# Lumina-Group/libzkp

Measured on AMD Instinct MI355X. Metric: proofs/sec (whole node) + ms/proof p50, 4096-proof mixed batch (range / equality / membership / improvement) per MI355X, higher is better.
Workload: dtype u32/u64 integer limbs (10x25.5-bit GF(2^255-19), BN254 Fq on 9x29-bit limbs in the MSM loops and 10x26-bit elsewhere, 8x32-bit Fr and scalars mod l, 2x64-bit f128)

## Files before the change

### libzkp_amd/csrc/g16_impl.inc

```

namespace {

struct G16Key {
    bool loaded = false;
    uint32_t n_inst = 0, n_wit = 0, nv = 0, n_rows = 0, m = 0, logm = 0;
    G16Circuit C{};
    std::vector<void*> allocs;
    uint32_t *table_g1 = nullptr, *table_g2 = nullptr;
    G16Radix rx = g16_radix(G16_WBITS_DEFAULT);
    int shared_tables = -1;
    uint64_t table_bytes = 0;
    struct Chunking { DevLayout lay; const uint32_t* corr = nullptr; const uint16_t* scal = nullptr; };
    std::vector<SlotList> targets_g1, targets_g2;
    std::vector<uint16_t> hscal_g1, hscal_g2;
    std::map<uint64_t, Chunking> lays_g1, lays_g2;
    uint64_t win_g1 = 0, win_g2 = 0;
    const uint32_t *init_g1 = nullptr, *init_g2 = nullptr;
    G16Vk vk{}; bool vk_ready = false;
    uint64_t vk_table_bytes = 0;
    bool verifier_only() const { return vk_ready && !loaded; }
    const uint32_t *vm_kconst = nullptr, *vm_lines = nullptr;
};
struct G16Run {
    void* buf = nullptr; size_t cap = 0; hipStream_t side = nullptr, side2 = nullptr; hipEvent_t ev[4] = {nullptr, nullptr, nullptr, nullptr};
    hipEvent_t last = nullptr; bool used = false;
};
struct G16State {
    G16Key key[2];
    uint32_t* mimc_dev = nullptr;
    G16Run run[2][2];
    bool attr_set = false;
    G16VmTables vm;
};
G16State& g16s() {
    if (!dev().g16) dev().g16 = new G16State();
    return *dev().g16;
}

template <class Tv> int dev_upload(G16Key& K, Tv** dst, const std::vector<typename std::remove_const<Tv>::type>& src) {
    typename std::remove_const<Tv>::type* p = nullptr;
    HIP_TRY(hipMalloc(&p, src.size() * sizeof(src[0]) + 16));
    if (!src.empty()) HIP_TRY(hipMemcpy(p, src.data(), src.size() * sizeof(src[0]), hipMemcpyHostToDevice));
// ... 42 lines not shown
template <class J> void append_words(std::vector<uint32_t>& v, const J& p) { const uint32_t* w = reinterpret_cast<const uint32_t*>(&p); for (size_t i = 0; i < sizeof(J) / 4; i++) v.push_back(w[i]); }
template <class J> J host_neg_multiple(const J& o, uint32_t k) {
    J acc = o; for (uint32_t i = 1; i < k; i++) acc = jac_add(acc, o);
    return jac_neg(acc);
}
void append_offset(std::vector<uint32_t>& v, bool g2, uint32_t k) {
    const MsmOffsets& o = msm_offsets();
    if (!g2) append_words(v, k ? host_neg_multiple(o.o1, k) : o.o1); else append_words(v, k ? host_neg_multiple(o.o2, k) : o.o2);
}
int upload_offset_point(G16Key& K, bool g2, const uint32_t** d_init) { std::vector<uint32_t> init; append_offset(init, g2, 0); return dev_upload(K, d_init, init); }
uint32_t choose_chunks(uint64_t windows, uint32_t ntargets, uint32_t rows, uint32_t resident, uint32_t tb) {
    const uint32_t groups = (rows + tb - 1) / tb;
    uint32_t hi = (uint32_t)(windows / 8); if (hi > 2048) hi = 2048; if (hi < ntargets) hi = ntargets;
    uint32_t best = ntargets; double best_cost = 1e300;
    for (uint32_t c = ntargets; c <= hi; c++) {
        const double rounds = std::ceil((double)c * groups / resident);
        const double cost = rounds * (std::ceil((double)windows / c) + 2.5) + 0.25 * c / 8.0;
        if (cost < best_cost) { best_cost = cost; best = c; }
    }
    return best;
}
int get_chunking(G16Key& K, bool g2, int part, uint32_t rows, const G16Key::Chunking** out) {
    const uint32_t resident = (uint32_t)dev().num_cu * g16_msm_blocks_per_cu(g2);
    if (part == G16_PART_ALL && !g2) return fail(ZKP_HIP_E_ARGUMENT, "G16_PART_ALL is the G2 launch");
    const std::vector<SlotList> targets = g16_part_targets(g2 ? K.targets_g2 : K.targets_g1, part);
    uint32_t c = choose_chunks(g16_windows(targets), (uint32_t)targets.size(), rows, resident, g16_msm_rows_per_block(g2));
    if (g_budget_request >= 10000) c = g_budget_request - 10000;
    auto& cache = g2 ? K.lays_g2 : K.lays_g1;
    const uint64_t key = (uint64_t)part << 32 | c;
    auto it = cache.find(key);
    if (it == cache.end()) {
        const G16Chunks P = g16_plan_chunks(targets, g2 ? K.hscal_g2 : K.hscal_g1, part, c);
        G16Key::Chunking ch; int rc;
        const GatherShape shape{K.rx.nent, K.rx.slot_ent, K.rx.uneven ? 1u : 0u, K.rx.digw};
        if ((rc = upload_layout(ch.lay, P.L, &shape, P.scal.data()))) return rc;
        std::vector<uint32_t> corr;
        for (uint32_t k : P.offsets) append_offset(corr, g2, k);
        if ((rc = dev_upload(K, &ch.corr, corr))) return rc;
        if ((rc = dev_upload(K, &ch.scal, P.scal))) return rc;
        it = cache.emplace(key, ch).first;
    }
    *out = &it->second;
    return 0;
}


uint64_t key_table_bytes(size_t n1, size_t n2, uint32_t wbits, bool uneven = false) {
    const G16Radix rx = g16_radix(wbits, uneven);
    return ((uint64_t)n1 * g16_table_entry_words(false, true) + (uint64_t)n2 * g16_table_entry_words(true, true)) * 4ull * rx.slot_ent;
}
int choose_radix(size_t n1, size_t n2, uint32_t* wbits_out, bool* uneven_out) {
    *uneven_out = false;
    const int forced = env_int("ZKP_HIP_G16_WBITS", 0);
    if (forced) {
        if (forced < (int)G16_WBITS_MIN || forced > (int)G16_WBITS_MAX) return fail(ZKP_HIP_E_ARGUMENT, "ZKP_HIP_G16_WBITS must be 8..15");
        *wbits_out = (uint32_t)forced; *uneven_out = forced == 14 && env_int("ZKP_HIP_G16_UNEVEN", 1) != 0; return 0;
    }
    size_t free_b = 0, total_b = 0;
    HIP_TRY(hipMemGetInfo(&free_b, &total_b));
    const int budget_mb = env_int("ZKP_HIP_G16_TABLE_BUDGET_MB", 0);
    const uint64_t reserve = 8ull << 30;
    const uint64_t fits = free_b > reserve ? (uint64_t)((free_b - reserve) * 0.45) : 0;
    uint64_t budget = budget_mb > 0 ? (uint64_t)budget_mb << 20 : fits;
    uint32_t first = G16_WBITS_KNEE;
    if (budget_mb > 0) {
        first = G16_WBITS_DEFAULT;
        if (G16_WBITS_DEFAULT == 14 && env_int("ZKP_HIP_G16_UNEVEN", 1) != 0 && key_table_bytes(n1, n2, 14, true) <= budget) { *wbits_out = 14; *uneven_out = true; return 0; }
    }
    for (uint32_t w = first; w >= G16_WBITS_MIN; w--)
        if (key_table_bytes(n1, n2, w) <= budget) { *wbits_out = w; return 0; }
    char msg[256];
    snprintf(msg, sizeof msg, "not enough device memory for the proving key's window tables: %llu MB at the smallest radix (2^%u), budget %llu MB (%llu MB free)",
             (unsigned long long)(key_table_bytes(n1, n2, G16_WBITS_MIN) >> 20), G16_WBITS_MIN, (unsigned long long)(budget >> 20), (unsigned long long)(free_b >> 20));
    return fail(ZKP_HIP_E_RUNTIME, msg);
}
struct SharedTables { int hip_dev, kind; uint8_t digest[32]; uint32_t wbits; bool share_ab; uint32_t *g1, *g2; int refs; };
struct TableRegistry { std::mutex mu; std::vector<SharedTables> v; std::map<int, std::mutex> build_mu; };
TableRegistry& table_registry() { static TableRegistry* r = new TableRegistry(); return *r; }
std::mutex& table_build_mutex(int hip_dev) { TableRegistry& R = table_registry(); std::lock_guard<std::mutex> lk(R.mu); return R.build_mu[hip_dev]; }
bool acquire_tables(G16Key& K, const SharedTables& want, bool any_radix) {
    TableRegistry& R = table_registry();
    std::lock_guard<std::mutex> lk(R.mu);
    for (size_t i = 0; i < R.v.size(); i++) {
        SharedTables& e = R.v[i];
        if (e.refs <= 0 || e.hip_dev != want.hip_dev || e.kind != want.kind || e.share_ab != want.share_ab || memcmp(e.digest, want.digest, 32) || (!any_radix && e.wbits != want.wbits)) continue;
        e.refs++; K.shared_tables = (int)i; K.table_g1 = e.g1; K.table_g2 = e.g2; K.rx = g16_radix(e.wbits & 0xffu, (e.wbits >> 8) != 0);
        return true;
    }
    return false;
}
void register_tables(G16Key& K, SharedTables e) {
    TableRegistry& R = table_registry();
    std::lock_guard<std::mutex> lk(R.mu);
    e.refs = 1; R.v.push_back(e);
    K.shared_tables = (int)R.v.size() - 1; K.table_g1 = e.g1; K.table_g2 = e.g2;
}
template <uint32_t AW, class Pt>
int build_tables(G16Key& K, const std::vector<Pt>& bases, uint32_t** table, bool msm_form, const G16Radix& rx, bool owned = true) {
    std::vector<uint32_t> flat; flat.reserve(bases.size() * AW);
    for (auto& b : bases) { const uint32_t* w = reinterpret_cast<const uint32_t*>(&b); for (uint32_t k = 0; k < AW; k++) flat.push_back(w[k]); }
    uint32_t* d_bases = nullptr; int rc;
    if ((rc = dev_upload(K, &d_bases, flat))) return rc;
    const size_t words = bases.size() * (size_t)rx.slot_ent * g16_table_entry_words(AW == 40, msm_form);
    uint32_t* tab = nullptr;
    if (hipMalloc(&tab, words * 4 + 64) != hipSuccess) {
        (void)hipGetLastError();
        char msg[200]; snprintf(msg, sizeof msg, "out of device memory allocating %llu MB of key tables (radix 2^%u)", (unsigned long long)((words * 4) >> 20), rx.wbits);
        return fail(ZKP_HIP_E_RUNTIME, msg);
    }
    if (owned) K.allocs.push_back(tab);
    g16_launch_build_table(AW == 40, d_bases, (uint32_t)bases.size(), tab, dev().stream, msm_form, rx);
    HIP_TRY(hipGetLastError());
    HIP_TRY(hipStreamSynchronize(dev().stream));
    *table = tab;
    return 0;
}

void release_key(G16Key& K) {
    (void)hipDeviceSynchronize();
    if (K.shared_tables >= 0) {
        TableRegistry& R = table_registry();
        std::lock_guard<std::mutex> lk(R.mu);
        SharedTables& e = R.v[(size_t)K.shared_tables];
        if (--e.refs == 0) { (void)hipFree(e.g1); (void)hipFree(e.g2); e.g1 = e.g2 = nullptr; }
    }
    for (void* p : K.allocs) (void)hipFree(p);
    for (auto& e : K.lays_g1) free_layout(e.second.lay);
    for (auto& e : K.lays_g2) free_layout(e.second.lay);
    K = G16Key();
}
int load_key_body(int kind, const uint8_t* pk, uint64_t len);
int no_proving_key(const G16Key& K) {
    return fail(ZKP_HIP_E_ARGUMENT, K.verifier_only() ? "only a verifying key is loaded for this circuit: proving needs the proving key (zkp_hip_groth16_load_key)"
                                                      : "no proving key loaded for this circuit (zkp_hip_groth16_load_key)");
}
int load_key_locked(int kind, const uint8_t* pk, uint64_t len) {
    if (kind != G16_EQUALITY && kind != G16_MEMBERSHIP) return fail(ZKP_HIP_E_ARGUMENT, "unknown circuit kind");
    G16Key& K = g16s().key[kind];
    if (K.loaded || K.shared_tables >= 0 || !K.allocs.empty()) release_key(K);
    int rc;
// ... 18 lines not shown
    K.vk.ml_alpha_beta = miller_loop(B.beta_g2.p, aff_neg(B.alpha_g1.p));
    std::vector<uint32_t> kc(6 * 20), lines;
    g16_vm_key_constants(B.beta_g2.p, aff_neg(B.alpha_g1.p), B.gamma_g2.p, B.delta_g2.p, kc.data(), lines);
    if ((rc = dev_upload(K, &K.vm_kconst, kc)) || (rc = dev_upload(K, &K.vm_lines, lines))) return rc;
    K.vk_ready = true;
    return 0;
}
int ensure_mimc_dev() {
    if (g16s().mimc_dev) return 0;
    ensure_mimc_constants();
    std::vector<uint32_t> mc; for (auto& c : g_mimc_host) put_fr(mc, c);
    HIP_TRY(hipMalloc(&g16s().mimc_dev, mc.size() * 4)); HIP_TRY(hipMemcpy(g16s().mimc_dev, mc.data(), mc.size() * 4, hipMemcpyHostToDevice));
    return 0;
}
int load_key_body(int kind, const uint8_t* pk, uint64_t len) {
    G16Key& K = g16s().key[kind];
    const HostR1CS cs = kind == G16_EQUALITY ? build_equality_r1cs() : build_membership_r1cs();
    int rc;
    KeyReader R{pk, len};
    G16VkBlob B; G16PkBlob Q;
    const int format = g16_read_key_prefix(R, B);
    if (format == G16_BLOB_MALFORMED)
        return fail(ZKP_HIP_E_ARGUMENT, "malformed proving key or verifying key (expected ark-serialize uncompressed ProvingKey<Bn254>, or its VerifyingKey<Bn254> alone)");
    if (format == G16_BLOB_VERIFYING_KEY) {
        if (const char* why = g16_check_verifying_key(B, cs.n_inst)) return fail(ZKP_HIP_E_ARGUMENT, why);
        return install_verifying_key(K, B);
    }
    if (const char* why = g16_read_proving_key(R, B, g16_key_shape(cs), Q)) return fail(ZKP_HIP_E_ARGUMENT, why);
    const bool share_ab = env_int("ZKP_HIP_G16_SHARE_AB", 1) != 0;
    G16KeyPlan P;
    if (const char* why = g16_plan_key(P, B, Q, cs, share_ab)) return fail(ZKP_HIP_E_UNSUPPORTED, why);
    SharedTables want{}; want.hip_dev = dev().hip_dev; want.kind = kind; want.share_ab = share_ab; sha256_host(want.digest, pk, len);
    std::lock_guard<std::mutex> build_lock(table_build_mutex(want.hip_dev));
    if (env_int("ZKP_HIP_G16_WBITS", 0) != 0 || !acquire_tables(K, want, true)) {
        uint32_t wb = 0; bool uneven = false;
        if ((rc = choose_radix(P.radix_points_g1, P.radix_points_g2, &wb, &uneven))) return rc;
        K.rx = g16_radix(wb, uneven); want.wbits = K.rx.wbits | K.rx.uneven << 8;
        if (!acquire_tables(K, want, false)) {
            if ((rc = build_tables<20>(K, P.bases_g1, &want.g1, true, K.rx, false))) return rc;
            if ((rc = build_tables<40>(K, P.bases_g2, &want.g2, true, K.rx, false))) { (void)hipFree(want.g1); return rc; }
            register_tables(K, want);
        }
    }
    K.table_bytes = key_table_bytes(P.bases_g1.size(), P.bases_g2.size(), K.rx.wbits, K.rx.uneven);
    if ((rc = upload_circuit(K, cs)) || (rc = ensure_mimc_dev())) return rc;
    K.targets_g1 = g16_plan_targets(P.cls_g1, K.rx); K.targets_g2 = g16_plan_targets(P.cls_g2, K.rx);
    K.win_g1 = g16_windows(K.targets_g1); K.win_g2 = g16_windows(K.targets_g2);
    K.hscal_g1 = P.row_g1; K.hscal_g2 = P.row_g2;
    if ((rc = upload_offset_point(K, false, &K.init_g1)) || (rc = upload_offset_point(K, true, &K.init_g2))) return rc;
    if (!g16_check_verifying_key(B, K.n_inst) && (rc = install_verifying_key(K, B))) return rc;
    K.loaded = true;
    return 0;
}


fr tape_fr(const uint32_t seed[8], uint32_t idx, uint32_t slot) { uint32_t w[16]; tape_draw64(w, seed, idx, slot); return fp_from_wide<FrParams>(w); }

MsmView g16_msm_view(const G16Radix& rx, const DevLayout& D, const uint16_t* slot_scalar, const uint32_t* table, const uint32_t* acc_init, uint32_t rows, const uint32_t* digits, uint32_t* partial) {
    MsmView m; m.nwin = rx.nwin; m.nent = rx.nent; m.digw = rx.digw; m.slot_ent = rx.slot_ent; m.uneven = rx.uneven; m.rows = rows; m.nslots = D.nslots; m.nchunks = D.nchunks; m.table = table; m.digits = digits;
    m.slot_base = D.slot_base; m.slot_scalar = slot_scalar; m.slot_nwin = D.slot_nwin; m.chunk_begin = D.chunk_begin; m.chunk_win0 = D.chunk_win0; m.chunk_nwin = D.chunk_nwin; m.partial = partial; m.acc_init = acc_init;
    m.steps = D.steps; m.chunk_step0 = D.chunk_step0;
    return m;
}

int gpu_scalar_mults(bool g2, const std::vector<fr>& scalars, std::vector<uint8_t>& out_bytes) {
    const uint32_t rows = (uint32_t)scalars.size(), AW = g2 ? 40 : 20, JW = g2 ? G2_JAC_W : G1_JAC_W, PB = g2 ? 128 : 64;
    std::vector<uint32_t> base;
    if (!g2) append_words(base, host_g1_generator()); else append_words(base, host_g2_generator());
    std::vector<uint32_t> offs; append_offset(offs, g2, 0); append_offset(offs, g2, 1);
    const G16Radix rx = g16_radix(10);
    std::vector<uint32_t> dig((size_t)rx.digw * rows);
    for (uint32_t i = 0; i < rows; i++) {
        sc raw; fp_to_raw(raw.v, scalars[i]); uint32_t pk[G16_DIGW_MAX]; g16_recode(pk, raw, rx);
        for (uint32_t k = 0; k < rx.digw; k++) dig[(size_t)k * rows + i] = pk[k];
    }
    uint32_t *d_base = nullptr, *d_tab = nullptr, *d_dig = nullptr, *d_part = nullptr, *d_offs = nullptr, *d_sums = nullptr; uint8_t* d_out = nullptr;
    DevScope mem;
    HIP_TRY(mem.alloc(&d_base, AW * 4)); HIP_TRY(mem.alloc(&d_tab, (size_t)rx.slot_ent * g16_table_entry_words(g2, true) * 4 + 64)); HIP_TRY(mem.alloc(&d_dig, dig.size() * 4));
    HIP_TRY(mem.alloc(&d_part, (size_t)JW * 4 * rows)); HIP_TRY(mem.alloc(&d_sums, (size_t)JW * 4 * rows)); HIP_TRY(mem.alloc(&d_offs, offs.size() * 4));
    HIP_TRY(hipMemcpy(d_offs, offs.data(), offs.size() * 4, hipMemcpyHostToDevice)); HIP_TRY(mem.alloc(&d_out, (size_t)PB * rows));
    HIP_TRY(hipMemcpy(d_base, base.data(), AW * 4, hipMemcpyHostToDevice));
// ... 64 lines not shown
    put_len(pk, nv); put(pk, g1at(o_a), 64ull * nv);
    put_len(pk, nv); put(pk, g1at(o_b), 64ull * nv);
    put_len(pk, nv); put(pk, g2at(3), 128ull * nv);
    put_len(pk, m - 1); put(pk, g1at(o_h), 64ull * (m - 1));
    put_len(pk, T.n_wit); put(pk, g1at(o_l), 64ull * T.n_wit);
    return load_key_locked(kind, pk.data(), pk.size());
}

int launch_msm_key(bool g2, const G16Radix& rx, const G16Key::Chunking& ch, const uint32_t* table, const uint32_t* acc_init, uint32_t rows, const uint32_t* digits, uint32_t* partial, hipStream_t st) {
    const DevLayout& D = ch.lay;
    const MsmView m = g16_msm_view(rx, D, ch.scal, table, acc_init, rows, digits, partial);
    Device::KProf& K = dev().prof[g2 ? 2 : 1];
    hipEvent_t e1 = nullptr;
    int rc = prof_begin(K, st, &e1);
    if (rc) return rc;
    ZKP_TRACED(g2 ? "k_msm_gather<G2Msm>" : "k_msm_gather<G1Msm>", st, g16_launch_msm(g2, m, st));
    prof_end(K, st, e1, D.adds_per_row * rows);
    return 0;
}


int run_g16(int kind, uint32_t rows, const uint64_t* d_value, const uint64_t* d_set_vals, const uint32_t* d_set_len, const uint8_t* d_seeds,
            uint8_t* d_out, uint64_t stride, hipStream_t st, uint32_t lane = 0) {
    G16Key& K = g16s().key[kind];
    if (!K.loaded) return no_proving_key(K);
    const uint32_t nsc = g16_nscalars(K.nv, K.m);
    const G16Key::Chunking *c1 = nullptr, *c1c = nullptr, *c2 = nullptr;
    int rc;
    if ((rc = get_chunking(K, false, G16_PART_AB, rows, &c1)) || (rc = get_chunking(K, true, G16_PART_ALL, rows, &c2))) return rc;
    if ((rc = get_chunking(K, false, G16_PART_C, rows, &c1c))) return rc;
    size_t off = 0;
    auto sz = [&](size_t bytes) { size_t o = off; off += align_up(bytes); return o; };
    const size_t W = (size_t)32 * rows;
    const size_t o_z = sz(W * K.nv), o_sd = sz((size_t)K.rx.digw * 4 * rows * nsc), o_rs = sz(W * 2), o_p1 = sz((size_t)c1->lay.nchunks * G1_JAC_W * 4 * rows),
                 o_p1c = sz((size_t)c1c->lay.nchunks * G1_JAC_W * 4 * rows), o_p2 = sz((size_t)c2->lay.nchunks * G2_JAC_W * 4 * rows),
                 o_s1 = sz((size_t)3 * G1_JAC_W * 4 * rows), o_s2 = sz((size_t)G2_JAC_W * 4 * rows), o_t1 = sz((size_t)G16_CPARTS * G1_JAC_W * 4 * rows),
                 o_qe = sz((size_t)2 * 9 * K.m * 4 * rows);
    G16Run& RW = g16s().run[kind][lane & 1u];
    if (off > RW.cap) {
        if (RW.buf) { HIP_TRY(hipDeviceSynchronize()); HIP_TRY(hipFree(RW.buf)); RW.buf = nullptr; RW.cap = 0; }
        HIP_TRY(hipMalloc(&RW.buf, off)); RW.cap = off;
    }
    uint8_t* base = (uint8_t*)RW.buf;
    G16View V{}; V.rx = K.rx; V.rows = rows; V.kind = (uint32_t)kind; V.n_inst = K.n_inst; V.n_wit = K.n_wit; V.nv = K.nv; V.m = K.m;
    V.value = d_value; V.set_vals = d_set_vals; V.set_len = d_set_len; V.seeds = reinterpret_cast<const uint32_t*>(d_seeds); V.mimc_c = g16s().mimc_dev;
    V.z = (uint32_t*)(base + o_z); V.sdig = (uint32_t*)(base + o_sd); V.rs = (uint32_t*)(base + o_rs); V.out = d_out; V.stride = stride;
    V.qap_evals = (uint32_t*)(base + o_qe);
    uint32_t *p1 = (uint32_t*)(base + o_p1), *p1c = (uint32_t*)(base + o_p1c), *p2 = (uint32_t*)(base + o_p2), *s1 = (uint32_t*)(base + o_s1), *s2 = (uint32_t*)(base + o_s2), *t1 = (uint32_t*)(base + o_t1);
    if (!RW.last) {
        for (auto& e : RW.ev) HIP_TRY(hipEventCreateWithFlags(&e, hipEventDisableTiming));
        HIP_TRY(hipEventCreateWithFlags(&RW.last, hipEventDisableTiming));
    }
    G16Run& R0 = g16s().run[kind][0];
    if (!R0.side) {
        static const int side_level = env_int("ZKP_HIP_G16_SIDE_PRIORITY", 2), side2_level = env_int("ZKP_HIP_G16_SIDE2_PRIORITY", 0);
        HIP_TRY(hipStreamCreateWithPriority(&R0.side, hipStreamNonBlocking, stream_priority(side_level)));
        HIP_TRY(hipStreamCreateWithPriority(&R0.side2, hipStreamNonBlocking, stream_priority(side2_level)));
    }
    hipStream_t const side = R0.side, side2 = R0.side2;
    hipEvent_t ev_wit = RW.ev[0], ev_ab = RW.ev[1], ev_c = RW.ev[2], ev_cp = RW.ev[3];
    ReduceView R2{}; R2.rows = rows; R2.ntargets = 1; R2.partial = p2; R2.target_chunk_begin = c2->lay.target_chunk_begin; R2.corr = c2->corr;
    if (RW.used) HIP_TRY(hipStreamWaitEvent(st, RW.last, 0));
    ZKP_TRACED("k_g16_witness", st, g16_launch_witness(V, st));
    ZKP_TRACED("k_g16_zdigits", st, g16_launch_zdigits(V, st));
    HIP_TRY(hipEventRecord(ev_wit, st));
    HIP_TRY(hipStreamWaitEvent(side, ev_wit, 0));
    { TraceMark tm_("k_g16_qap", side); HIP_TRY(g16_launch_qap(V, K.C, side)); }
    if ((rc = launch_msm_key(false, K.rx, *c1c, K.table_g1, K.init_g1, rows, V.sdig, p1c, side))) return rc;
    ReduceView Rc{}; Rc.rows = rows; Rc.ntargets = 1; Rc.partial = p1c; Rc.target_chunk_begin = c1c->lay.target_chunk_begin; Rc.corr = c1c->corr;
    ZKP_TRACED("k_sum_t<G1Msm>", side, g16_launch_sum(false, Rc, s1 + (size_t)2 * G1_JAC_W * rows, side));
    HIP_TRY(hipEventRecord(ev_c, side));
    if ((rc = launch_msm_key(false, K.rx, *c1, K.table_g1, K.init_g1, rows, V.sdig, p1, st))) return rc;
    ReduceView Rab{}; Rab.rows = rows; Rab.ntargets = 2; Rab.partial = p1; Rab.target_chunk_begin = c1->lay.target_chunk_begin; Rab.corr = c1->corr;
    if (c1->lay.ntargets == 3) Rab.target_chunk_end = c1->lay.target_chunk_begin + 2;
    HIP_TRY(hipEventRecord(ev_ab, st));
    HIP_TRY(hipStreamWaitEvent(side2, ev_ab, 0));
    ZKP_TRACED("k_sum_t<G1Msm>", side2, g16_launch_sum(false, Rab, s1, side2));
    ZKP_TRACED("k_g16_cparts", side2, g16_launch_cparts(V, s1, t1, side2));
    HIP_TRY(hipEventRecord(ev_cp, side2));
    if ((rc = launch_msm_key(true, K.rx, *c2, K.table_g2, K.init_g2, rows, V.sdig, p2, st))) return rc;
    ZKP_TRACED("k_sum_t<G2Msm>", st, g16_launch_sum(true, R2, s2, st));
    HIP_TRY(hipStreamWaitEvent(st, ev_c, 0));
    HIP_TRY(hipStreamWaitEvent(st, ev_cp, 0));
    ZKP_TRACED("k_g16_final", st, g16_launch_final(V, s1, s2, t1, st));
    HIP_TRY(hipGetLastError());
    HIP_TRY(hipEventRecord(RW.last, st)); RW.used = true;
    return 0;
}

int prove_g16_host(int kind, uint64_t n, const uint64_t* values, const uint64_t* sets_flat, const uint32_t* set_counts, const std::vector<uint8_t>& valid,
                   const uint8_t* seeds, uint8_t* out, uint64_t stride, uint32_t* out_len, int32_t* status) {
    if (g16s().key[kind].verifier_only()) return no_proving_key(g16s().key[kind]);
    std::vector<uint64_t> v, sv; std::vector<uint32_t> sl, idx; std::vector<uint8_t> sd;
    size_t pos = 0; int any = 0;
    memset(out, 0, stride * n);
    for (uint64_t i = 0; i < n; i++) {
        const uint32_t cnt = set_counts ? set_counts[i] : 0;
        if (valid[i]) {
            idx.push_back((uint32_t)i); v.push_back(values[i]);
            sd.insert(sd.end(), seeds + 32 * i, seeds + 32 * i + 32);
            if (kind == G16_MEMBERSHIP) { sl.push_back(cnt); for (uint32_t k = 0; k < G16_MAX_SET; k++) sv.push_back(k < cnt ? sets_flat[pos + k] : 0); }
            const uint32_t plen = kind == G16_EQUALITY ? 298u : 10u + 4u + 8u * cnt + 256u + 32u;
            if (plen > stride) return fail(ZKP_HIP_E_ARGUMENT, "stride too small for the proof envelope");
            out_len[i] = plen; status[i] = ZKP_HIP_OK;
        } else { out_len[i] = 0; status[i] = ZKP_HIP_INVALID_INPUT; any = 1; }
        pos += cnt;
    }
    const uint32_t rows = (uint32_t)idx.size();
    if (rows == 0) return any;
    hipStream_t st = dev().stream;
    uint64_t *d_v = nullptr, *d_sv = nullptr; uint32_t* d_sl = nullptr; uint8_t *d_sd = nullptr, *d_out = nullptr;
    DevScope mem;
    HIP_TRY(mem.alloc(&d_v, 8ull * rows)); HIP_TRY(mem.alloc(&d_sd, 32ull * rows)); HIP_TRY(mem.alloc(&d_out, stride * rows));
// ... 291 lines not shown
```

### libzkp_amd/csrc/g16_share.h

```cpp
#pragma once
#include <cstdint>
#include <vector>
#include "bp_layout.h"
#include "g16_circuit.h"
#include "g16_keyblob.h"

namespace zkp {

inline bool g16_shared_point(const G1Pt& a, const G1Pt& b) { return !a.inf && !b.inf && fq_eq(a.p.x, b.p.x) && fq_eq(a.p.y, b.p.y); }

struct G16AbSlots { SlotList a, s, b; };
inline G16AbSlots g16_ab_slots(const std::vector<G1Pt>& aq, const std::vector<G1Pt>& b1q, const std::vector<uint8_t>& cls, bool share) {
    G16AbSlots out;
    const size_t n = aq.size() < b1q.size() ? aq.size() : b1q.size();
    for (size_t k = 0; k < aq.size(); k++) {
        if (aq[k].inf) continue;
        if (share && k < n && g16_shared_point(aq[k], b1q[k])) out.s.push_back({(uint16_t)k, cls[k]});
        else out.a.push_back({(uint16_t)k, cls[k]});
    }
    for (size_t k = 0; k < b1q.size(); k++) {
        if (b1q[k].inf || (share && k < n && g16_shared_point(aq[k], b1q[k]))) continue;
        out.b.push_back({(uint16_t)k, cls[k]});
    }
    return out;
// ... 22 lines not shown
    const G16KeyShape sh = g16_key_shape(cs);
    if (sh.nv + sh.m + 3 > 65535 || 3ull * sh.nv + sh.m + 8 > 65535) return "circuit too large for 16-bit slot indices";
    const uint32_t SC_H = sh.nv, SC_R = sh.nv + sh.m - 1, SC_S = SC_R + 1, SC_NRS = SC_R + 2, SC_ONE = SC_R + 3;
    std::vector<uint8_t> cls(cs.inst_nwin); cls.insert(cls.end(), cs.wit_nwin.begin(), cs.wit_nwin.end());
    P = G16KeyPlan(); P.cls_g1.resize(4); P.cls_g2.resize(1);
    auto add1 = [&](int list, const G1Pt& pt, uint32_t row, uint8_t c) {
        if (pt.inf) return;
        P.cls_g1[list].push_back({(uint16_t)P.bases_g1.size(), c}); P.bases_g1.push_back(pt.p); P.row_g1.push_back((uint16_t)row);
    };
    auto add2 = [&](const G2Pt& pt, uint32_t row, uint8_t c) {
        if (pt.inf) return;
        P.cls_g2[0].push_back({(uint16_t)P.bases_g2.size(), c}); P.bases_g2.push_back(pt.p); P.row_g2.push_back((uint16_t)row);
    };
    const G16AbSlots ab = g16_ab_slots(pk.a_query, pk.b_g1_query, cls, share_ab);
    for (auto& sl : ab.a) add1(0, pk.a_query[sl.first], sl.first, sl.second);
    add1(0, pk.delta_g1, SC_R, G16_NW_FULL); add1(0, vk.alpha_g1, SC_ONE, 1);
    for (auto& sl : ab.s) add1(1, pk.a_query[sl.first], sl.first, sl.second);
    for (auto& sl : ab.b) add1(2, pk.b_g1_query[sl.first], sl.first, sl.second);
    add1(2, pk.delta_g1, SC_S, G16_NW_FULL); add1(2, pk.beta_g1, SC_ONE, 1);
    for (uint32_t k = 0; k < sh.n_wit; k++) add1(3, pk.l_query[k], sh.n_inst + k, cls[sh.n_inst + k]);
    for (uint32_t i = 0; i + 1 < sh.m; i++) add1(3, pk.h_query[i], SC_H + i, G16_NW_FULL);
    add1(3, pk.delta_g1, SC_NRS, G16_NW_FULL);
    for (uint32_t k = 0; k < sh.nv; k++) add2(pk.b_g2_query[k], k, cls[k]);
    add2(vk.delta_g2, SC_S, G16_NW_FULL); add2(vk.beta_g2, SC_ONE, 1);
    P.radix_points_g1 = pk.a_query.size() + pk.b_g1_query.size() - ab.s.size() + pk.l_query.size() + pk.h_query.size() + 5;
    P.radix_points_g2 = pk.b_g2_query.size() + 2;
    return nullptr;
}
inline std::vector<SlotList> g16_plan_targets(const std::vector<SlotList>& cls, const G16Radix& rx) {
    std::vector<SlotList> out = cls;
    for (auto& t : out) for (auto& sl : t) sl.second = g16_class_nwin(sl.second, rx);
    return out;
}
inline uint64_t g16_windows(const std::vector<SlotList>& targets) { uint64_t w = 0; for (auto& t : targets) for (auto& sl : t) w += sl.second; return w; }

enum { G16_PART_ALL = 0, G16_PART_AB = 1, G16_PART_C = 2 };
inline std::vector<SlotList> g16_part_targets(const std::vector<SlotList>& all, int part) {
    if (part == G16_PART_ALL) return all;
    if (part == G16_PART_AB) return g16_ab_targets(all[0], all[1], all[2]);
    return std::vector<SlotList>(all.begin() + 3, all.end());
}
struct G16Chunks { MsmLayout L; std::vector<uint16_t> scal; std::vector<uint32_t> offsets; };
inline G16Chunks g16_plan_chunks(const std::vector<SlotList>& targets, const std::vector<uint16_t>& row, int part, uint32_t chunks) {
    G16Chunks C; C.L = make_layout_even(targets, chunks);
    for (uint16_t b : C.L.slot_base) C.scal.push_back(row[b]);
    if (part == G16_PART_AB) { const G16AbRanges ab = g16_ab_ranges(C.L); for (int t = 0; t < 2; t++) C.offsets.push_back((uint32_t)ab.end[t] - ab.begin[t]); }
    else for (uint32_t t = 0; t < C.L.ntargets(); t++) C.offsets.push_back((uint32_t)C.L.target_chunk_begin[t + 1] - C.L.target_chunk_begin[t]);
    return C;
}

}
```

### libzkp_amd/csrc/g16_steps.h

```cpp
#pragma once
#include "bn254_g.h"
#include "bn254_fr9.h"
#include "keccak.h"
#include "sc25519.h"

namespace zkp {

struct G16Radix { uint32_t wbits, nwin, nent, digw, nwin_u64, uneven, slot_ent; };
constexpr uint32_t G16_UNEVEN_TOP_ENT = 25088;
ZKP_HD inline G16Radix g16_radix(uint32_t wbits, bool uneven = false) {
    G16Radix r; r.wbits = wbits; r.nwin = (254 + wbits) / wbits; r.nent = 1u << (wbits - 1); r.nwin_u64 = (64 + wbits) / wbits; r.uneven = 0;
    r.slot_ent = r.nwin * r.nent;
    if (uneven && wbits == 14) { r.uneven = 1; r.nwin = 18; r.slot_ent = 18u * r.nent + G16_UNEVEN_TOP_ENT; }
    r.digw = (r.nwin + 1) / 2;
    return r;
}
ZKP_HD inline uint32_t g16_win_bit(const G16Radix& rx, uint32_t w) { return rx.uneven && w == 17 ? 239u : rx.wbits * w; }
ZKP_HD inline uint32_t g16_win_off(const G16Radix& rx, uint32_t w) { return (w + (rx.uneven && w == 17 ? 1u : 0u)) * rx.nent; }
ZKP_HD inline uint32_t g16_win_ent(const G16Radix& rx, uint32_t w) { return !rx.uneven || w < 16 ? rx.nent : w == 16 ? 2u * rx.nent : G16_UNEVEN_TOP_ENT; }
constexpr uint32_t G16_WBITS_DEFAULT = 14, G16_WBITS_KNEE = 13, G16_WBITS_MIN = 8, G16_WBITS_MAX = 15, G16_DIGW_MAX = 16;
static_assert(G16_WBITS_DEFAULT >= G16_WBITS_MIN && G16_WBITS_DEFAULT <= G16_WBITS_MAX, "key-table radix out of range");
ZKP_HD inline void g16_recode_uneven(uint32_t* packed, const sc& raw) {
    uint32_t carry = 0;
    ZKP_UNROLL for (int j = 0; j < 18; j++) {
        const int bit = j == 17 ? 239 : 14 * j, wb = j < 16 ? 14 : 15, wd = bit >> 5, sh = bit & 31;
        uint32_t x = wd < 8 ? raw.v[wd] >> sh : 0u;
        if (sh + wb > 32 && wd + 1 < 8) x |= raw.v[wd + 1] << (32 - sh);
        uint32_t d = (x & ((1u << wb) - 1u)) + carry;
        carry = j < 17 && d > (1u << (wb - 1)) ? 1u : 0u;
        d = (d - (carry << wb)) & 0xffffu;
        if ((j & 1) == 0) packed[j >> 1] = d; else packed[j >> 1] |= d << 16;
    }
}
ZKP_HD inline void g16_recode(uint32_t* packed, const sc& raw, const G16Radix& rx) {
    if (rx.uneven) { g16_recode_uneven(packed, raw); return; }
    switch (rx.wbits) {
        case 8: sc_recode_signed<8, 32>(packed, raw); break;
        case 9: sc_recode_signed<9, 29>(packed, raw); break;
        case 10: sc_recode_signed<10, 26>(packed, raw); break;
        case 11: sc_recode_signed<11, 24>(packed, raw); break;
        case 12: sc_recode_signed<12, 22>(packed, raw); break;
        case 13: sc_recode_signed<13, 20>(packed, raw); break;
        case 14: sc_recode_signed<14, 19>(packed, raw); break;
        default: sc_recode_signed<15, 17>(packed, raw); break;
    }
}
constexpr uint32_t G16V_WBITS = 10, G16V_NWIN = 26, G16V_NENT = 512, G16V_NWIN_U64 = 7;

constexpr uint32_t MIMC_ROUNDS = 110, G16_MAX_SET = 64;
constexpr uint32_t G16_TAPE_IDX = 0x47313600u;
enum { G16_EQUALITY = 0, G16_MEMBERSHIP = 1 };

ZKP_HD inline fr ld_fr(const uint32_t* p, uint32_t idx, uint32_t row, uint32_t rows) {
    fr r; const uint32_t* q = p + (size_t)idx * 8 * rows + row;
    ZKP_UNROLL for (int k = 0; k < 8; k++) r.v[k] = q[(size_t)k * rows];
    return r;
}
ZKP_HD inline void st_fr(uint32_t* p, uint32_t idx, uint32_t row, uint32_t rows, const fr& s) {
    uint32_t* q = p + (size_t)idx * 8 * rows + row;
    ZKP_UNROLL for (int k = 0; k < 8; k++) q[(size_t)k * rows] = s.v[k];
}
ZKP_HD inline fr ld_fr_c(const uint32_t* p, uint32_t idx) { fr r; ZKP_UNROLL for (int k = 0; k < 8; k++) r.v[k] = p[(size_t)idx * 8 + k]; return r; }
ZKP_HD inline void g16_put_bytes(uint8_t* dst, const uint32_t* w, int nwords) {
    for (int i = 0; i < nwords; i++) { dst[4 * i] = (uint8_t)w[i]; dst[4 * i + 1] = (uint8_t)(w[i] >> 8); dst[4 * i + 2] = (uint8_t)(w[i] >> 16); dst[4 * i + 3] = (uint8_t)(w[i] >> 24); }
}
ZKP_HD inline void st_fr_digits(uint32_t* d, uint32_t idx, uint32_t row, uint32_t rows, const fr& x, const G16Radix& rx) {
    sc raw; fp_to_raw(raw.v, x);
    uint32_t pk[G16_DIGW_MAX]; g16_recode(pk, raw, rx);
    uint32_t* q = d + (size_t)idx * rx.digw * rows + row;
    ZKP_UNROLL for (uint32_t k = 0; k < G16_DIGW_MAX; k++) if (k < rx.digw) q[(size_t)k * rows] = pk[k];
}

struct G16View {
    uint32_t rows, kind;
    G16Radix rx;
    uint32_t n_inst, n_wit, nv, m;
    const uint64_t* value;
    const uint64_t* set_vals;
    const uint32_t* set_len;
    const uint32_t* seeds;
    const uint32_t* mimc_c;
    uint32_t* z;
    uint32_t* sdig;
    uint32_t* rs;
    uint32_t* qap_evals;
    uint8_t* out; uint64_t stride;
};
ZKP_HD inline uint32_t g16_sc_h(const G16View& V) { return V.nv; }
ZKP_HD inline uint32_t g16_sc_r(const G16View& V) { return V.nv + V.m - 1; }
ZKP_HD inline uint32_t g16_sc_s(const G16View& V) { return V.nv + V.m; }
ZKP_HD inline uint32_t g16_sc_nrs(const G16View& V) { return V.nv + V.m + 1; }
ZKP_HD inline uint32_t g16_sc_one(const G16View& V) { return V.nv + V.m + 2; }
ZKP_HD inline uint32_t g16_nscalars(uint32_t nv, uint32_t m) { return nv + m + 3; }

ZKP_HD inline fr g16_mimc_chain(const G16View& V, uint32_t row, fr x, uint32_t wit0) {
    for (uint32_t i = 0; i < MIMC_ROUNDS; i++) {
        const fr t = fp_add(x, ld_fr_c(V.mimc_c, i));
        const fr t2 = fp_sq(t), t4 = fp_sq(t2);
        x = fp_mul(t4, t);
        if (V.z) { st_fr(V.z, wit0 + 3 * i, row, V.rows, t2); st_fr(V.z, wit0 + 3 * i + 1, row, V.rows, t4); st_fr(V.z, wit0 + 3 * i + 2, row, V.rows, x); }
    }
    return x;
}

ZKP_HD inline void step_g16_witness(const G16View& V, uint32_t row) {
    const uint32_t rows = V.rows;
    const uint64_t val = V.value[row];
    const fr one = fp_one<FrParams>(), zero = fp_zero<FrParams>();
    const fr v = fp_from_u64<FrParams>(val);
    uint8_t* o = V.out + (uint64_t)row * V.stride;
    st_fr(V.z, 0, row, rows, one);
    fr h;
    uint32_t proof_len = 256;
    if (V.kind == G16_EQUALITY) {
        st_fr(V.z, 2, row, rows, v); st_fr(V.z, 3, row, rows, v);
        h = g16_mimc_chain(V, row, v, 4);
// ... 7 lines not shown
        h = g16_mimc_chain(V, row, v, w0 + 1);
        st_fr(V.z, 1, row, rows, h);
        uint32_t pos = 0xffffffffu;
        for (uint32_t i = 0; i < len; i++) if (pos == 0xffffffffu && sv[i] == val) pos = i;
        const uint32_t sel0 = w0 + 1 + 3 * MIMC_ROUNDS;
        for (uint32_t i = 0; i < G16_MAX_SET; i++) {
            const bool real = i < len;
            const fr si = fp_from_u64<FrParams>(real ? sv[i] : 0);
            st_fr(V.z, 2 + i, row, rows, si);
            st_fr(V.z, 2 + G16_MAX_SET + i, row, rows, real ? one : zero);
            const bool sel = i == pos;
            st_fr(V.z, sel0 + i, row, rows, sel ? one : zero);
            st_fr(V.z, sel0 + G16_MAX_SET + i, row, rows, (sel && !real) ? one : zero);
            st_fr(V.z, sel0 + 2 * G16_MAX_SET + i, row, rows, sel ? fp_sub(v, si) : zero);
        }
        o[0] = 2; o[1] = 4;
        proof_len = 4 + 8 * len + 256;
        uint8_t* pl = o + 10;
        pl[0] = (uint8_t)len; pl[1] = (uint8_t)(len >> 8); pl[2] = (uint8_t)(len >> 16); pl[3] = (uint8_t)(len >> 24);
        for (uint32_t i = 0; i < len; i++) for (int k = 0; k < 8; k++) pl[4 + 8 * i + k] = (uint8_t)(sv[i] >> (8 * k));
    }
    for (int k = 0; k < 4; k++) { o[2 + k] = (uint8_t)(proof_len >> (8 * k)); o[6 + k] = (uint8_t)(32u >> (8 * k)); }
    uint32_t hraw[8]; fp_to_raw(hraw, h);
    g16_put_bytes(o + 10 + proof_len, hraw, 8);
    uint32_t seed[8]; ZKP_UNROLL for (int k = 0; k < 8; k++) seed[k] = V.seeds[(size_t)row * 8 + k];
    uint32_t w[16];
    tape_draw64(w, seed, G16_TAPE_IDX, 0); const fr r = fp_from_wide<FrParams>(w);
    tape_draw64(w, seed, G16_TAPE_IDX, 1); const fr s = fp_from_wide<FrParams>(w);
    st_fr_digits(V.sdig, g16_sc_r(V), row, rows, r, V.rx);
    st_fr_digits(V.sdig, g16_sc_s(V), row, rows, s, V.rx);
    st_fr_digits(V.sdig, g16_sc_nrs(V), row, rows, fp_neg(fp_mul(r, s)), V.rx);
    uint32_t* q = V.sdig + (size_t)g16_sc_one(V) * V.rx.digw * rows + row;
    q[0] = 1u; for (uint32_t k = 1; k < V.rx.digw; k++) q[(size_t)k * rows] = 0u;
    fr rr, sr; fp_to_raw(rr.v, r); fp_to_raw(sr.v, s);
    st_fr(V.rs, 0, row, rows, rr); st_fr(V.rs, 1, row, rows, sr);
}
ZKP_HD inline void step_g16_zdigits(const G16View& V, uint32_t k, uint32_t row) {
    st_fr_digits(V.sdig, k, row, V.rows, ld_fr(V.z, k, row, V.rows), V.rx);
}

struct G16Circuit {
    uint32_t n_rows, m, logm;
    const uint32_t *a_ptr, *a_col, *a_coef, *b_ptr, *b_col, *b_coef, *c_ptr, *c_col, *c_coef;
    const uint32_t *tw, *tw_inv;
    const uint32_t *coset, *coset_inv;
    const uint32_t* zinv;
};
ZKP_HD inline fr g16_row_dot(const uint32_t* ptr, const uint32_t* col, const uint32_t* coef, uint32_t r, const uint32_t* z, uint32_t row, uint32_t rows) {
    fr acc = fp_zero<FrParams>();
    for (uint32_t e = ptr[r]; e < ptr[r + 1]; e++) acc = fp_add(acc, fp_mul(ld_fr_c(coef, e), ld_fr(z, col[e], row, rows)));
    return acc;
}
ZKP_HD inline uint32_t g16_bitrev(uint32_t x, uint32_t bits) {
    uint32_t r = 0; for (uint32_t i = 0; i < bits; i++) { r = (r << 1) | (x & 1u); x >>= 1; } return r;
}

struct G16Lds {
    uint32_t* base; uint32_t m;
    ZKP_HD static uint32_t sw(uint32_t e) { return e ^ ((0u - ((e >> 5) & 1u)) & 10u) ^ ((0u - ((e >> 6) & 1u)) & 21u); }
    ZKP_HD fr9 ld(uint32_t e) const { fr9 r; const uint32_t p = sw(e); ZKP_UNROLL for (int k = 0; k < 9; k++) r.v[k] = base[(size_t)k * m + p]; return r; }
    ZKP_HD void st(uint32_t e, const fr9& v) const { const uint32_t p = sw(e); ZKP_UNROLL for (int k = 0; k < 9; k++) base[(size_t)k * m + p] = v.v[k]; }
};
ZKP_HD inline fr9 ld_fr9_c(const uint32_t* p, uint32_t idx) { fr9 r; ZKP_UNROLL for (int k = 0; k < 9; k++) r.v[k] = p[(size_t)idx * 9 + k]; return r; }
ZKP_HD inline fr g16_row_dot_fast(const uint32_t* ptr, const uint32_t* col, const uint32_t* coef, uint32_t r, const uint32_t* z, uint32_t row, uint32_t rows) {
    const fr one = fp_one<FrParams>();
    fr acc = fp_zero<FrParams>();
    for (uint32_t e = ptr[r]; e < ptr[r + 1]; e++) {
        const fr cf = ld_fr_c(coef, e);
        const uint32_t c = col[e];
        bool is_one = true; ZKP_UNROLL for (int k = 0; k < 8; k++) is_one = is_one && cf.v[k] == one.v[k];
        if (c == 0) acc = fp_add(acc, cf);
// ... 136 lines not shown
```

Baseline: 339,200.

## Give the G2 MSM its own wider window radix, separate from G1

The G2 key tables can now use a wider signed-digit radix than G1. By default it picks 2^13 to 2^15, taken only when the tables fit in about 10% of free device memory; env variables can force it or cap it. When the two radices differ, the prover keeps a second scalar-digit buffer and a variable-to-G2-row map, and writes recoded digits for both radices during the z-digit and r/s steps. The aim is fewer windows, so fewer bucket additions in the expensive G2 MSM. The cost is larger G2 tables, more device memory, extra digit recoding and stores, and a registry key that now encodes both radices.

```diff
diff --git a/libzkp_amd/csrc/g16_impl.inc b/libzkp_amd/csrc/g16_impl.inc
--- a/libzkp_amd/csrc/g16_impl.inc
+++ b/libzkp_amd/csrc/g16_impl.inc
@@ -8,6 +8,9 @@
     std::vector<void*> allocs;
     uint32_t *table_g1 = nullptr, *table_g2 = nullptr;
     G16Radix rx = g16_radix(G16_WBITS_DEFAULT);
+    G16Radix rx2 = g16_radix(G16_WBITS_DEFAULT);
+    bool split() const { return !g16_same_radix(rx, rx2); }
+    const uint16_t* g2row = nullptr; uint32_t g2_s = G16_NO_ROW, g2_one = G16_NO_ROW;
     int shared_tables = -1;
     uint64_t table_bytes = 0;
     struct Chunking { DevLayout lay; const uint32_t* corr = nullptr; const uint16_t* scal = nullptr; };
@@ -116,7 +119,8 @@
     if (it == cache.end()) {
         const G16Chunks P = g16_plan_chunks(targets, g2 ? K.hscal_g2 : K.hscal_g1, part, c);
         G16Key::Chunking ch; int rc;
-        const GatherShape shape{K.rx.nent, K.rx.slot_ent, K.rx.uneven ? 1u : 0u, K.rx.digw};
+        const G16Radix& rx = g2 ? K.rx2 : K.rx;
+        const GatherShape shape{rx.nent, rx.slot_ent, rx.uneven ? 1u : 0u, rx.digw};
         if ((rc = upload_layout(ch.lay, P.L, &shape, P.scal.data()))) return rc;
         std::vector<uint32_t> corr;
         for (uint32_t k : P.offsets) append_offset(corr, g2, k);
@@ -129,12 +133,15 @@
 }
 
 
+uint64_t key_table_bytes(size_t n1, size_t n2, const G16Radix& rx, const G16Radix& rx2) {
+    return g16_group_table_bytes(n1, g16_table_entry_words(false, true), rx) + g16_group_table_bytes(n2, g16_table_entry_words(true, true), rx2);
+}
 uint64_t key_table_bytes(size_t n1, size_t n2, uint32_t wbits, bool uneven = false) {
     const G16Radix rx = g16_radix(wbits, uneven);
-    return ((uint64_t)n1 * g16_table_entry_words(false, true) + (uint64_t)n2 * g16_table_entry_words(true, true)) * 4ull * rx.slot_ent;
-}
-int choose_radix(size_t n1, size_t n2, uint32_t* wbits_out, bool* uneven_out) {
-    *uneven_out = false;
+    return key_table_bytes(n1, n2, rx, rx);
+}
+int choose_radix(size_t n1, size_t n2, uint32_t* wbits_out, bool* uneven_out, bool* whole_key, uint64_t* free_out) {
+    *uneven_out = false; *whole_key = true; *free_out = 0;
     const int forced = env_int("ZKP_HIP_G16_WBITS", 0);
     if (forced) {
         if (forced < (int)G16_WBITS_MIN || forced > (int)G16_WBITS_MAX) return fail(ZKP_HIP_E_ARGUMENT, "ZKP_HIP_G16_WBITS must be 8..15");
@@ -142,6 +149,7 @@
     }
     size_t free_b = 0, total_b = 0;
     HIP_TRY(hipMemGetInfo(&free_b, &total_b));
+    *free_out = free_b; *whole_key = env_int("ZKP_HIP_G16_TABLE_BUDGET_MB", 0) > 0;
     const int budget_mb = env_int("ZKP_HIP_G16_TABLE_BUDGET_MB", 0);
     const uint64_t reserve = 8ull << 30;
     const uint64_t fits = free_b > reserve ? (uint64_t)((free_b - reserve) * 0.45) : 0;
@@ -154,11 +162,26 @@
     for (uint32_t w = first; w >= G16_WBITS_MIN; w--)
         if (key_table_bytes(n1, n2, w) <= budget) { *wbits_out = w; return 0; }
     char msg[256];
-    snprintf(msg, sizeof msg, "not enough device memory for the proving key's window tables: %llu MB at the smallest radix (2^%u), budget %llu MB (%llu MB free)",
+    snprintf(msg, sizeof msg, "not enough device memory for the proving key's G1 and G2 window tables: %llu MB at the smallest radix (2^%u), budget %llu MB (%llu MB free)",
              (unsigned long long)(key_table_bytes(n1, n2, G16_WBITS_MIN) >> 20), G16_WBITS_MIN, (unsigned long long)(budget >> 20), (unsigned long long)(free_b >> 20));
     return fail(ZKP_HIP_E_RUNTIME, msg);
 }
+int choose_g2_radix(const G16Radix& g1, size_t n2, bool whole_key, uint64_t free_b, G16Radix* out) {
+    const int forced = env_int("ZKP_HIP_G16_G2_WBITS", 0);
+    if (forced) {
+        if (forced < (int)G16_WBITS_MIN || forced > (int)G16_G2_WBITS_MAX) return fail(ZKP_HIP_E_ARGUMENT, "ZKP_HIP_G16_G2_WBITS must be 8..16");
+        *out = (uint32_t)forced == g1.wbits ? g1 : g16_radix((uint32_t)forced); return 0;
+    }
+    *out = g1;
+    if (whole_key) return 0;
+    const int budget_mb = env_int("ZKP_HIP_G16_G2_TABLE_BUDGET_MB", 0);
+    const uint64_t reserve = 8ull << 30;
+    const uint64_t budget = budget_mb > 0 ? (uint64_t)budget_mb << 20 : free_b > reserve ? (uint64_t)((free_b - reserve) * G16_G2_FREE_SHARE) : 0;
+    *out = g16_choose_g2_radix(g1, n2, g16_table_entry_words(true, true), budget, G16_G2_WBITS_AUTO_MAX);
+    return 0;
+}
 struct SharedTables { int hip_dev, kind; uint8_t digest[32]; uint32_t wbits; bool share_ab; uint32_t *g1, *g2; int refs; };
+uint32_t registry_radix(const G16Radix& rx, const G16Radix& rx2) { return rx.wbits | rx.uneven << 8 | rx2.wbits << 16 | rx2.uneven << 24; }
 struct TableRegistry { std::mutex mu; std::vector<SharedTables> v; std::map<int, std::mutex> build_mu; };
 TableRegistry& table_registry() { static TableRegistry* r = new TableRegistry(); return *r; }
 std::mutex& table_build_mutex(int hip_dev) { TableRegistry& R = table_registry(); std::lock_guard<std::mutex> lk(R.mu); return R.build_mu[hip_dev]; }
@@ -168,7 +191,7 @@
     for (size_t i = 0; i < R.v.size(); i++) {
         SharedTables& e = R.v[i];
         if (e.refs <= 0 || e.hip_dev != want.hip_dev || e.kind != want.kind || e.share_ab != want.share_ab || memcmp(e.digest, want.digest, 32) || (!any_radix && e.wbits != want.wbits)) continue;
-        e.refs++; K.shared_tables = (int)i; K.table_g1 = e.g1; K.table_g2 = e.g2; K.rx = g16_radix(e.wbits & 0xffu, (e.wbits >> 8) != 0);
+        e.refs++; K.shared_tables = (int)i; K.table_g1 = e.g1; K.table_g2 = e.g2; K.rx = g16_radix(e.wbits & 0xffu, ((e.wbits >> 8) & 0xffu) != 0); K.rx2 = g16_radix((e.wbits >> 16) & 0xffu, (e.wbits >> 24) != 0);
         return true;
     }
     return false;
@@ -180,7 +203,7 @@
     K.shared_tables = (int)R.v.size() - 1; K.table_g1 = e.g1; K.table_g2 = e.g2;
 }
 template <uint32_t AW, class Pt>
-int build_tables(G16Key& K, const std::vector<Pt>& bases, uint32_t** table, bool msm_form, const G16Radix& rx, bool owned = true) {
+int build_tables(G16Key& K, const std::vector<Pt>& bases, uint32_t** table, bool msm_form, const G16Radix& rx, bool owned = true, const char* group = "G1") {
     std::vector<uint32_t> flat; flat.reserve(bases.size() * AW);
     for (auto& b : bases) { const uint32_t* w = reinterpret_cast<const uint32_t*>(&b); for (uint32_t k = 0; k < AW; k++) flat.push_back(w[k]); }
     uint32_t* d_bases = nullptr; int rc;
@@ -189,7 +212,7 @@
     uint32_t* tab = nullptr;
     if (hipMalloc(&tab, words * 4 + 64) != hipSuccess) {
         (void)hipGetLastError();
-        char msg[200]; snprintf(msg, sizeof msg, "out of device memory allocating %llu MB of key tables (radix 2^%u)", (unsigned long long)((words * 4) >> 20), rx.wbits);
+        char msg[200]; snprintf(msg, sizeof msg, "out of device memory allocating %llu MB of %s key tables (radix 2^%u)", (unsigned long long)((words * 4) >> 20), group, rx.wbits);
         return fail(ZKP_HIP_E_RUNTIME, msg);
     }
     if (owned) K.allocs.push_back(tab);
@@ -274,21 +297,28 @@
     if (const char* why = g16_plan_key(P, B, Q, cs, share_ab)) return fail(ZKP_HIP_E_UNSUPPORTED, why);
     SharedTables want{}; want.hip_dev = dev().hip_dev; want.kind = kind; want.share_ab = share_ab; sha256_host(want.digest, pk, len);
     std::lock_guard<std::mutex> build_lock(table_build_mutex(want.hip_dev));
-    if (env_int("ZKP_HIP_G16_WBITS", 0) != 0 || !acquire_tables(K, want, true)) {
-        uint32_t wb = 0; bool uneven = false;
-        if ((rc = choose_radix(P.radix_points_g1, P.radix_points_g2, &wb, &uneven))) return rc;
-        K.rx = g16_radix(wb, uneven); want.wbits = K.rx.wbits | K.rx.uneven << 8;
+    if (env_int("ZKP_HIP_G16_WBITS", 0) != 0 || env_int("ZKP_HIP_G16_G2_WBITS", 0) != 0 || !acquire_tables(K, want, true)) {
+        uint32_t wb = 0; bool uneven = false, whole_key = true; uint64_t free_b = 0;
+        if ((rc = choose_radix(P.radix_points_g1, P.radix_points_g2, &wb, &uneven, &whole_key, &free_b))) return rc;
+        K.rx = g16_radix(wb, uneven);
+        if ((rc = choose_g2_radix(K.rx, P.bases_g2.size(), whole_key, free_b, &K.rx2))) return rc;
+        want.wbits = registry_radix(K.rx, K.rx2);
         if (!acquire_tables(K, want, false)) {
-            if ((rc = build_tables<20>(K, P.bases_g1, &want.g1, true, K.rx, false))) return rc;
-            if ((rc = build_tables<40>(K, P.bases_g2, &want.g2, true, K.rx, false))) { (void)hipFree(want.g1); return rc; }
+            if ((rc = build_tables<20>(K, P.bases_g1, &want.g1, true, K.rx, false, "G1"))) return rc;
+            if ((rc = build_tables<40>(K, P.bases_g2, &want.g2, true, K.rx2, false, "G2"))) { (void)hipFree(want.g1); return rc; }
             register_tables(K, want);
         }
     }
-    K.table_bytes = key_table_bytes(P.bases_g1.size(), P.bases_g2.size(), K.rx.wbits, K.rx.uneven);
+    K.table_bytes = key_table_bytes(P.bases_g1.size(), P.bases_g2.size(), K.rx, K.rx2);
     if ((rc = upload_circuit(K, cs)) || (rc = ensure_mimc_dev())) return rc;
-    K.targets_g1 = g16_plan_targets(P.cls_g1, K.rx); K.targets_g2 = g16_plan_targets(P.cls_g2, K.rx);
+    const G16G2Launch G2 = g16_plan_g2_launch(P, K.rx, K.rx2, K.nv, K.m);
+    K.targets_g1 = g16_plan_targets(P.cls_g1, K.rx); K.targets_g2 = G2.targets;
     K.win_g1 = g16_windows(K.targets_g1); K.win_g2 = g16_windows(K.targets_g2);
-    K.hscal_g1 = P.row_g1; K.hscal_g2 = P.row_g2;
+    K.hscal_g1 = P.row_g1; K.hscal_g2 = G2.slot_row;
+    if (G2.own_rows) {
+        K.g2_s = G2.rows.row_s; K.g2_one = G2.rows.row_one;
+        if ((rc = dev_upload(K, &K.g2row, G2.rows.row_of_var))) return rc;
+    }
     if ((rc = upload_offset_point(K, false, &K.init_g1)) || (rc = upload_offset_point(K, true, &K.init_g2))) return rc;
     if (!g16_check_verifying_key(B, K.n_inst) && (rc = install_verifying_key(K, B))) return rc;
     K.loaded = true;
@@ -419,7 +449,8 @@
     size_t off = 0;
     auto sz = [&](size_t bytes) { size_t o = off; off += align_up(bytes); return o; };
     const size_t W = (size_t)32 * rows;
-    const size_t o_z = sz(W * K.nv), o_sd = sz((size_t)K.rx.digw * 4 * rows * nsc), o_rs = sz(W * 2), o_p1 = sz((size_t)c1->lay.nchunks * G1_JAC_W * 4 * rows),
+    const bool split = K.split();
+    const size_t o_z = sz(W * K.nv), o_sd = sz((size_t)K.rx.digw * 4 * rows * nsc), o_sd2 = split ? sz((size_t)K.rx2.digw * 4 * rows * K.hscal_g2.size()) : 0, o_rs = sz(W * 2), o_p1 = sz((size_t)c1->lay.nchunks * G1_JAC_W * 4 * rows),
                  o_p1c = sz((size_t)c1c->lay.nchunks * G1_JAC_W * 4 * rows), o_p2 = sz((size_t)c2->lay.nchunks * G2_JAC_W * 4 * rows),
                  o_s1 = sz((size_t)3 * G1_JAC_W * 4 * rows), o_s2 = sz((size_t)G2_JAC_W * 4 * rows), o_t1 = sz((size_t)G16_CPARTS * G1_JAC_W * 4 * rows),
                  o_qe = sz((size_t)2 * 9 * K.m * 4 * rows);
@@ -433,6 +464,7 @@
     V.value = d_value; V.set_vals = d_set_vals; V.set_len = d_set_len; V.seeds = reinterpret_cast<const uint32_t*>(d_seeds); V.mimc_c = g16s().mimc_dev;
     V.z = (uint32_t*)(base + o_z); V.sdig = (uint32_t*)(base + o_sd); V.rs = (uint32_t*)(base + o_rs); V.out = d_out; V.stride = stride;
     V.qap_evals = (uint32_t*)(base + o_qe);
+    V.rx2 = K.rx2; V.sdig2 = split ? (uint32_t*)(base + o_sd2) : nullptr; V.g2row = K.g2row; V.g2_s = K.g2_s; V.g2_one = K.g2_one;
     uint32_t *p1 = (uint32_t*)(base + o_p1), *p1c = (uint32_t*)(base + o_p1c), *p2 = (uint32_t*)(base + o_p2), *s1 = (uint32_t*)(base + o_s1), *s2 = (uint32_t*)(base + o_s2), *t1 = (uint32_t*)(base + o_t1);
     if (!RW.last) {
         for (auto& e : RW.ev) HIP_TRY(hipEventCreateWithFlags(&e, hipEventDisableTiming));
@@ -465,7 +497,7 @@
     ZKP_TRACED("k_sum_t<G1Msm>", side2, g16_launch_sum(false, Rab, s1, side2));
     ZKP_TRACED("k_g16_cparts", side2, g16_launch_cparts(V, s1, t1, side2));
     HIP_TRY(hipEventRecord(ev_cp, side2));
-    if ((rc = launch_msm_key(true, K.rx, *c2, K.table_g2, K.init_g2, rows, V.sdig, p2, st))) return rc;
+    if ((rc = launch_msm_key(true, K.rx2, *c2, K.table_g2, K.init_g2, rows, split ? V.sdig2 : V.sdig, p2, st))) return rc;
     ZKP_TRACED("k_sum_t<G2Msm>", st, g16_launch_sum(true, R2, s2, st));
     HIP_TRY(hipStreamWaitEvent(st, ev_c, 0));
     HIP_TRY(hipStreamWaitEvent(st, ev_cp, 0));
diff --git a/libzkp_amd/csrc/g16_share.h b/libzkp_amd/csrc/g16_share.h
--- a/libzkp_amd/csrc/g16_share.h
+++ b/libzkp_amd/csrc/g16_share.h
@@ -78,6 +78,32 @@
     for (auto& t : out) for (auto& sl : t) sl.second = g16_class_nwin(sl.second, rx);
     return out;
 }
+inline bool g16_same_radix(const G16Radix& a, const G16Radix& b) { return a.wbits == b.wbits && a.uneven == b.uneven; }
+inline uint64_t g16_group_table_bytes(size_t n, uint32_t entry_words, const G16Radix& rx) { return (uint64_t)n * entry_words * 4ull * rx.slot_ent; }
+struct G16G2Rows { std::vector<uint16_t> slot_row, row_of_var; uint32_t row_s = G16_NO_ROW, row_one = G16_NO_ROW; };
+inline G16G2Rows g16_plan_g2_rows(const G16KeyPlan& P, uint32_t nv, uint32_t m) {
+    G16G2Rows R; R.row_of_var.assign(nv, G16_NO_ROW);
+    const uint32_t SC_S = nv + m, SC_ONE = nv + m + 2;
+    for (size_t b = 0; b < P.row_g2.size(); b++) {
+        const uint32_t row = P.row_g2[b];
+        R.slot_row.push_back((uint16_t)b);
+        if (row < nv) R.row_of_var[row] = (uint16_t)b; else if (row == SC_S) R.row_s = (uint32_t)b; else if (row == SC_ONE) R.row_one = (uint32_t)b;
+    }
+    return R;
+}
+struct G16G2Launch { bool own_rows = false; std::vector<SlotList> targets; std::vector<uint16_t> slot_row; G16G2Rows rows; };
+inline G16G2Launch g16_plan_g2_launch(const G16KeyPlan& P, const G16Radix& rx, const G16Radix& rx2, uint32_t nv, uint32_t m) {
+    G16G2Launch L; L.own_rows = !g16_same_radix(rx, rx2);
+    L.targets = g16_plan_targets(P.cls_g2, rx2); L.slot_row = P.row_g2;
+    if (L.own_rows) { L.rows = g16_plan_g2_rows(P, nv, m); L.slot_row = L.rows.slot_row; }
+    return L;
+}
+constexpr double G16_G2_FREE_SHARE = 0.10;
+inline G16Radix g16_choose_g2_radix(const G16Radix& g1, size_t n2, uint32_t entry_words, uint64_t budget, uint32_t wmax = G16_G2_WBITS_MAX) {
+    for (uint32_t w = wmax; w >= G16_G2_WBITS_AUTO_MIN && w > g1.wbits; w--)
+        if (g16_group_table_bytes(n2, entry_words, g16_radix(w)) + (uint64_t)n2 * 40u * 4u <= budget) return g16_radix(w);
+    return g1;
+}
 inline uint64_t g16_windows(const std::vector<SlotList>& targets) { uint64_t w = 0; for (auto& t : targets) for (auto& sl : t) w += sl.second; return w; }
 
 enum { G16_PART_ALL = 0, G16_PART_AB = 1, G16_PART_C = 2 };
diff --git a/libzkp_amd/csrc/g16_steps.h b/libzkp_amd/csrc/g16_steps.h
--- a/libzkp_amd/csrc/g16_steps.h
+++ b/libzkp_amd/csrc/g16_steps.h
@@ -19,6 +19,8 @@
 ZKP_HD inline uint32_t g16_win_off(const G16Radix& rx, uint32_t w) { return (w + (rx.uneven && w == 17 ? 1u : 0u)) * rx.nent; }
 ZKP_HD inline uint32_t g16_win_ent(const G16Radix& rx, uint32_t w) { return !rx.uneven || w < 16 ? rx.nent : w == 16 ? 2u * rx.nent : G16_UNEVEN_TOP_ENT; }
 constexpr uint32_t G16_WBITS_DEFAULT = 14, G16_WBITS_KNEE = 13, G16_WBITS_MIN = 8, G16_WBITS_MAX = 15, G16_DIGW_MAX = 16;
+constexpr uint32_t G16_G2_WBITS_MAX = 16, G16_G2_WBITS_AUTO_MIN = 13, G16_G2_WBITS_AUTO_MAX = 15;
+constexpr uint16_t G16_NO_ROW = 0xffffu;
 static_assert(G16_WBITS_DEFAULT >= G16_WBITS_MIN && G16_WBITS_DEFAULT <= G16_WBITS_MAX, "key-table radix out of range");
 ZKP_HD inline void g16_recode_uneven(uint32_t* packed, const sc& raw) {
     uint32_t carry = 0;
@@ -42,7 +44,8 @@
         case 12: sc_recode_signed<12, 22>(packed, raw); break;
         case 13: sc_recode_signed<13, 20>(packed, raw); break;
         case 14: sc_recode_signed<14, 19>(packed, raw); break;
-        default: sc_recode_signed<15, 17>(packed, raw); break;
+        case 15: sc_recode_signed<15, 17>(packed, raw); break;
+        default: sc_recode_signed65536(packed, raw); break;
     }
 }
 constexpr uint32_t G16V_WBITS = 10, G16V_NWIN = 26, G16V_NENT = 512, G16V_NWIN_U64 = 7;
@@ -64,11 +67,14 @@
 ZKP_HD inline void g16_put_bytes(uint8_t* dst, const uint32_t* w, int nwords) {
     for (int i = 0; i < nwords; i++) { dst[4 * i] = (uint8_t)w[i]; dst[4 * i + 1] = (uint8_t)(w[i] >> 8); dst[4 * i + 2] = (uint8_t)(w[i] >> 16); dst[4 * i + 3] = (uint8_t)(w[i] >> 24); }
 }
-ZKP_HD inline void st_fr_digits(uint32_t* d, uint32_t idx, uint32_t row, uint32_t rows, const fr& x, const G16Radix& rx) {
-    sc raw; fp_to_raw(raw.v, x);
+ZKP_HD inline void st_raw_digits(uint32_t* d, uint32_t idx, uint32_t row, uint32_t rows, const sc& raw, const G16Radix& rx) {
     uint32_t pk[G16_DIGW_MAX]; g16_recode(pk, raw, rx);
     uint32_t* q = d + (size_t)idx * rx.digw * rows + row;
     ZKP_UNROLL for (uint32_t k = 0; k < G16_DIGW_MAX; k++) if (k < rx.digw) q[(size_t)k * rows] = pk[k];
+}
+ZKP_HD inline void st_fr_digits(uint32_t* d, uint32_t idx, uint32_t row, uint32_t rows, const fr& x, const G16Radix& rx) {
+    sc raw; fp_to_raw(raw.v, x);
+    st_raw_digits(d, idx, row, rows, raw, rx);
 }
 
 struct G16View {
@@ -82,6 +88,10 @@
     const uint32_t* mimc_c;
     uint32_t* z;
     uint32_t* sdig;
+    G16Radix rx2;
+    uint32_t* sdig2;
+    const uint16_t* g2row;
+    uint32_t g2_s, g2_one;
     uint32_t* rs;
     uint32_t* qap_evals;
     uint8_t* out; uint64_t stride;
@@ -155,11 +165,20 @@
     st_fr_digits(V.sdig, g16_sc_nrs(V), row, rows, fp_neg(fp_mul(r, s)), V.rx);
     uint32_t* q = V.sdig + (size_t)g16_sc_one(V) * V.rx.digw * rows + row;
     q[0] = 1u; for (uint32_t k = 1; k < V.rx.digw; k++) q[(size_t)k * rows] = 0u;
+    if (V.sdig2) {
+        if (V.g2_s != G16_NO_ROW) st_fr_digits(V.sdig2, V.g2_s, row, rows, s, V.rx2);
+        if (V.g2_one != G16_NO_ROW) {
+            uint32_t* q2 = V.sdig2 + (size_t)V.g2_one * V.rx2.digw * rows + row;
+            q2[0] = 1u; for (uint32_t k = 1; k < V.rx2.digw; k++) q2[(size_t)k * rows] = 0u;
+        }
+    }
     fr rr, sr; fp_to_raw(rr.v, r); fp_to_raw(sr.v, s);
     st_fr(V.rs, 0, row, rows, rr); st_fr(V.rs, 1, row, rows, sr);
 }
 ZKP_HD inline void step_g16_zdigits(const G16View& V, uint32_t k, uint32_t row) {
-    st_fr_digits(V.sdig, k, row, V.rows, ld_fr(V.z, k, row, V.rows), V.rx);
+    sc raw; fp_to_raw(raw.v, ld_fr(V.z, k, row, V.rows));
+    st_raw_digits(V.sdig, k, row, V.rows, raw, V.rx);
+    if (V.sdig2) { const uint32_t r2 = V.g2row[k]; if (r2 != G16_NO_ROW) st_raw_digits(V.sdig2, r2, row, V.rows, raw, V.rx2); }
 }
 
 struct G16Circuit {
```

Result: faster. 345,500 (median of 6 runs) (+1.9%).
